# bluenote-1577/sylph

Measured on AMD Instinct MI355X. Metric: read Gbp/s sketched + genome-comparisons/s profiled, 1 Gbp vs GTDB-R220, higher is better.
Workload: dtype u64

## Files before the change

### sylph_amd/csrc/capi.hip

```cpp
#include <algorithm>
#include <memory>

#include <thread>

#include "common.h"

namespace sylph {

static thread_local char g_err[1024] = "";

void set_error(const char* fmt, ...) {
    va_list ap;
    va_start(ap, fmt);
    vsnprintf(g_err, sizeof(g_err), fmt, ap);
    va_end(ap);
}

ScopedKernelTimer::ScopedKernelTimer(sylph_ctx* c, const char* family) : ctx(c), fam(family) {
    if (!ctx->profile) return;
    if (!ctx->profile_only.empty()) {
        const size_t n = strlen(family);
        size_t at = 0;
        bool found = false;
        while ((at = ctx->profile_only.find(family, at)) != std::string::npos) {
// ... 372 lines not shown
    sylph::ctx_unref(ctx);
}

int sylph_ctx_set_option(sylph_ctx* ctx, const char* key, const char* value) {
    return guarded([&] {
        SY_REQUIRE(ctx && key && value, "null argument");
        std::lock_guard<std::mutex> lock(ctx->mu);
        if (!strcmp(key, "finish")) {
            if (!strcmp(value, "auto")) ctx->finish_mode = 0;
            else if (!strcmp(value, "generic")) ctx->finish_mode = 1;
            else if (!strcmp(value, "bucket")) ctx->finish_mode = 2;
            else SY_REQUIRE(false, "finish must be auto|generic|bucket");
        } else if (!strcmp(key, "seeds")) {
            if (!strcmp(value, "auto") || !strcmp(value, "ordered")) ctx->seeds_mode = 0;
            else if (!strcmp(value, "unordered")) ctx->seeds_mode = 1;
            else if (!strcmp(value, "slots")) ctx->seeds_mode = 2;
            else SY_REQUIRE(false, "seeds must be auto|slots|unordered");
        } else if (!strcmp(key, "bucket_target")) {
            const long v = strtol(value, nullptr, 10);
            SY_REQUIRE(v >= 16 && v <= 256, "bucket_target must be in [16, 256]");
            ctx->bucket_target = (uint32_t)v;
        } else if (!strcmp(key, "plain_records")) {
            ctx->plain_records = (uint32_t)strtol(value, nullptr, 10) ? 1u : 0u;
        } else if (!strcmp(key, "shard_reduce")) {
            if (!strcmp(value, "alltoall")) ctx->shard_reduce = 0;
            else if (!strcmp(value, "allgather")) ctx->shard_reduce = 1;
            else SY_REQUIRE(false, "shard_reduce must be alltoall|allgather");
        } else if (!strcmp(key, "stream_priority")) {
            SY_REQUIRE(ctx->own_stream, "stream_priority: the context runs on the caller's stream");
            int least = 0, greatest = 0;
            DeviceGuard dg(ctx->device);
            SY_HIP(hipDeviceGetStreamPriorityRange(&least, &greatest));
            int prio = 0;
            if (!strcmp(value, "high")) prio = greatest;
            else if (!strcmp(value, "low")) prio = least;
            else SY_REQUIRE(!strcmp(value, "normal"), "stream_priority must be high|normal|low");
            SY_HIP(hipStreamSynchronize(ctx->stream));
            hipStream_t s = nullptr;
            SY_HIP(hipStreamCreateWithPriority(&s, hipStreamNonBlocking, prio));
            (void)hipStreamDestroy(ctx->stream);
            ctx->stream = s;
        } else if (!strcmp(key, "fail_next_peer_copy")) {
            ctx->fail_next_peer_copy = (uint32_t)strtol(value, nullptr, 10);
        } else if (!strcmp(key, "fail_next_shard_probe")) {
            ctx->fail_next_shard_probe = (uint32_t)strtol(value, nullptr, 10);
        } else if (!strcmp(key, "push_chunk_bytes")) {
            const long long v = strtoll(value, nullptr, 10);
            SY_REQUIRE(v >= 64 && v <= (1ll << 31), "push_chunk_bytes must be in [64, 2^31]");
            ctx->push_chunk_bytes = (uint64_t)v;
        } else if (!strcmp(key, "reads_wg_per_cu")) {
            const long v = strtol(value, nullptr, 10);
            SY_REQUIRE(v >= 0 && v <= 64, "reads_wg_per_cu must be in [0, 64]");
            ctx->reads_wg_per_cu = (uint32_t)v;
        } else if (!strcmp(key, "profile_only")) {
            ctx->profile_only = (!value[0] || !strcmp(value, "all")) ? std::string() : "," + std::string(value) + ",";
        } else if (!strcmp(key, "reads_tail_pct")) {
            const long v = strtol(value, nullptr, 10);
            SY_REQUIRE(v >= 0 && v <= 50, "reads_tail_pct must be in [0, 50]");
            ctx->reads_tail_pct = (uint32_t)v;
        } else if (!strcmp(key, "reads_hash")) {
            const long v = strtol(value, nullptr, 10);
            SY_REQUIRE(v >= -1 && v <= 2, "reads_hash must be -1 (default), 0, 1 or 2");
            ctx->reads_hash = (int)v;
        } else if (!strcmp(key, "reads_slack")) {
            ctx->reads_slack = (uint32_t)strtoul(value, nullptr, 0);
        } else if (!strcmp(key, "index_lambda")) {
            const long v = strtol(value, nullptr, 10);
            SY_REQUIRE(v >= 1 && v <= 8, "index_lambda must be in [1, 8]");
            ctx->index_lambda = (uint32_t)v;
        } else if (!strcmp(key, "cu_mask")) {
            SY_REQUIRE(ctx->own_stream, "cu_mask: the context runs on a caller-supplied stream");
            int cus = 256;
            (void)hipDeviceGetAttribute(&cus, hipDeviceAttributeMultiprocessorCount, ctx->device);
            long lo = 0, hi = cus;
            if (strcmp(value, "all")) {
                char* end = nullptr;
                lo = strtol(value, &end, 10);
                SY_REQUIRE(end && *end == ':', "cu_mask must be lo:hi or all");
                hi = strtol(end + 1, nullptr, 10);
            }
            SY_REQUIRE(lo >= 0 && lo < hi && hi <= cus, "cu_mask range [%ld, %ld) outside the device's %d CUs", lo, hi, cus);
            DeviceGuard dg(ctx->device);
            SY_HIP(hipStreamSynchronize(ctx->stream));
            std::vector<uint32_t> mask((size_t)(cus + 31) / 32, 0u);
            for (long i = lo; i < hi; i++) mask[(size_t)i >> 5] |= 1u << (i & 31);
            hipStream_t ns = nullptr;
            SY_HIP(hipExtStreamCreateWithCUMask(&ns, (uint32_t)mask.size(), mask.data()));
            (void)hipStreamDestroy(ctx->stream);
            ctx->stream = ns;
        } else if (!strcmp(key, "index_pass_max")) {
            const long long v = strtoll(value, nullptr, 10);
            SY_REQUIRE(v >= 1 && v <= (1ll << 31), "index_pass_max must be in [1, 2^31]");
            ctx->index_pass_max = (uint64_t)v;
        } else {
            SY_REQUIRE(false, "unknown option %s", key);
        }
    });
}

int sylph_ctx_profile(sylph_ctx* ctx, int enable) {
    return guarded([&] {
        SY_REQUIRE(ctx, "null ctx");
        std::lock_guard<std::mutex> lock(ctx->mu);
        profile_collect(ctx);
        ctx->stats.clear();
        ctx->profile = enable != 0;
// ... 16 lines not shown
```

### sylph_amd/csrc/common.h

```cpp
#pragma once
#include <hip/hip_runtime.h>

#include <atomic>
#include <cstdarg>
#include <cstdint>
#include <cstdio>
#include <cstdlib>
#include <cstring>
#include <ctime>
#include <map>
#include <mutex>
#include <string>
#include <vector>

#include "../../include/sylph_hip.h"

struct sylph_ctx;

namespace sylph {

void set_error(const char* fmt, ...);

struct HipError { hipError_t e; const char* what; const char* file; int line; };

// ... 70 lines not shown
    void alloc(size_t want) {
        if (ctx) p = pool_acquire(ctx, want, &cap);
        else { SY_HIP(hipMalloc(&p, want)); cap = want; }
    }
    void reserve(size_t bytes) {
        if (bytes <= cap) return;
        release();
        alloc(bytes + bytes / 4 + 256);
    }
    void grow_keep(size_t bytes, size_t keep, hipStream_t s) {
        if (bytes <= cap) return;
        void* old = p;
        const size_t old_cap = cap;
        p = nullptr;
        cap = 0;
        alloc(bytes * 2 + 256);
        if (keep && old) SY_HIP(hipMemcpyAsync(p, old, keep, hipMemcpyDeviceToDevice, s));
        if (old) {
            if (ctx) pool_release(ctx, old, old_cap);
            else { SY_HIP(hipStreamSynchronize(s)); (void)hipFree(old); }
        }
    }
    template <class T> T* as() const { return reinterpret_cast<T*>(p); }
};

struct KernelStat { double ms = 0; uint64_t launches = 0; };

}

#ifndef SYLPH_READS_TAIL_PCT
#define SYLPH_READS_TAIL_PCT 10
#endif
struct sylph_ctx {
    int device = 0;
    hipStream_t stream = nullptr;
    bool own_stream = false;
    std::mutex mu;
    int finish_mode = 0;
    uint32_t bucket_target = 128;
    uint32_t plain_records = 1;
    uint32_t shard_reduce = 0;
    uint32_t fail_next_peer_copy = 0;
    uint32_t fail_next_shard_probe = 0;
    uint32_t index_lambda = 0;
    uint64_t index_pass_max = 1ull << 30;
    struct SeedTurn { hipEvent_t gate = nullptr, done = nullptr; bool recorded = false; } turn;
    void seed_gate() { if (turn.gate) { (void)hipStreamWaitEvent(stream, turn.gate, 0); turn.gate = nullptr; } }
    void seed_done() { if (turn.done && !turn.recorded && hipEventRecord(turn.done, stream) == hipSuccess) turn.recorded = true; }
    std::string profile_only;
    uint32_t reads_tail_pct = SYLPH_READS_TAIL_PCT;
    int reads_hash = -1;
    uint32_t reads_slack = 0;
    uint32_t reads_wg_per_cu = 0;
    uint64_t push_chunk_bytes = 64ull << 20;
    int seeds_mode = 0;
    std::atomic<int> refs{1};
    bool profile = false;
    std::map<std::string, sylph::KernelStat> stats;
    struct Pending { std::string fam; hipEvent_t a, b; };
    std::vector<Pending> pending;
    std::vector<hipEvent_t> event_pool;
    std::vector<std::pair<size_t, void*>> pool_free;
    size_t pool_bytes = 0;
    sylph::DevBuf tmp_sort;
    sylph::DevBuf scratch[8];
    sylph::DevBuf counters;
    void* pinned = nullptr;
    void read_back(void* dst, const void* dev_src, size_t bytes);
    static constexpr size_t STAGE_BYTES = 32u << 20;
    void* stage[2] = {nullptr, nullptr};
    hipEvent_t stage_ev[2] = {nullptr, nullptr};
    hipStream_t copy_stream = nullptr;
    hipEvent_t copy_ev[2] = {nullptr, nullptr};
    void d2h(void* dst, const void* dev_src, size_t bytes);
    void h2d(void* dev_dst, const void* src, size_t bytes);
};

namespace sylph {

struct ScopedKernelTimer {
    sylph_ctx* ctx;
    hipEvent_t a = nullptr, b = nullptr;
    const char* fam;
    ScopedKernelTimer(sylph_ctx* c, const char* family);
    ~ScopedKernelTimer();
};
void profile_collect(sylph_ctx* ctx);
void ctx_unref(sylph_ctx* ctx);

struct HostPhase {
    sylph_ctx* ctx;
    const char* name;
    double t0 = 0;
    static bool enabled() { static const bool e = getenv("SYLPH_HIP_TRACE") != nullptr; return e; }
    static double now() { timespec ts; clock_gettime(CLOCK_MONOTONIC, &ts); return ts.tv_sec * 1e3 + ts.tv_nsec * 1e-6; }
    HostPhase(sylph_ctx* c, const char* n) : ctx(c), name(n) { if (enabled()) { (void)hipStreamSynchronize(c->stream); t0 = now(); } }
    ~HostPhase() { if (enabled()) { (void)hipStreamSynchronize(ctx->stream); fprintf(stderr, "[sylph_hip] %-28s %8.3f ms\n", name, now() - t0); } }
};

struct DeviceGuard {
    int prev = -1;
    explicit DeviceGuard(int dev) {
        (void)hipGetDevice(&prev);
        if (prev != dev) SY_HIP(hipSetDevice(dev));
        else prev = -1;
    }
    ~DeviceGuard() { if (prev >= 0) (void)hipSetDevice(prev); }
};

void sort_pairs_u64_u32(sylph_ctx* ctx, const uint64_t* kin, uint64_t* kout, const uint32_t* vin, uint32_t* vout,
                        size_t n, int begin_bit, int end_bit);
void sort_pairs_u32_u64(sylph_ctx* ctx, const uint32_t* kin, uint32_t* kout, const uint64_t* vin, uint64_t* vout,
                        size_t n, int begin_bit, int end_bit);
void sort_pairs_u32_u32(sylph_ctx* ctx, const uint32_t* kin, uint32_t* kout, const uint32_t* vin, uint32_t* vout,
                        size_t n, int begin_bit, int end_bit);
constexpr uint32_t SPILL_MAX_TILES = 256;
struct SpillState { uint32_t n_tiles; uint32_t tiles[SPILL_MAX_TILES]; };
struct ReadsState { uint32_t long_record; SpillState spill; };

void sort_keys_u32(sylph_ctx* ctx, const uint32_t* kin, uint32_t* kout, size_t n, int begin_bit, int end_bit);
void sort_keys_u64(sylph_ctx* ctx, const uint64_t* kin, uint64_t* kout, size_t n, int begin_bit, int end_bit);
void exclusive_sum_u32(sylph_ctx* ctx, const uint32_t* in, uint32_t* out, size_t n);
void inclusive_max_u32(sylph_ctx* ctx, const uint32_t* in, uint32_t* out, size_t n);

inline int bit_length(uint64_t v) { int b = 0; while (v) { b++; v >>= 1; } return b; }

}
```

### sylph_amd/csrc/reads.hip

```cpp
#include <cstddef>

#include "common.h"
#include "device_common.h"
#include "sketch_session.h"

namespace sylph {

namespace {

constexpr int RTPB = 256;
constexpr int RT_MIN = 4096, RT_MAX = 65536;
constexpr int RH = 400;
constexpr int RPAD = 32;
constexpr int MASKW = 12;
constexpr int OFFS_256 = 600;
constexpr int RTPB_RAGGED = 512;

template <int K>
struct KC {
    static constexpr uint64_t MASK = (1ull << (2 * K)) - 1;
};

__device__ __forceinline__ uint64_t win64(const uint32_t* sF, uint32_t b) {
    const uint32_t j = b >> 4, ph = (b & 15u) * 2u;
// ... 28 lines not shown
    else { fhi = __builtin_amdgcn_alignbit(A0, A1, 32 - 2 * T); flo = __builtin_amdgcn_alignbit(A1, A2, 32 - 2 * T); }
    constexpr int OFF = 2 * T - D;
    if constexpr (OFF < 0) { rlo = __builtin_amdgcn_alignbit(B0, Bm, OFF + 32); rhi = __builtin_amdgcn_alignbit(B1, B0, OFF + 32); }
    else if constexpr (OFF == 0) { rlo = B0; rhi = B1; }
    else { rlo = __builtin_amdgcn_alignbit(B1, B0, OFF); rhi = __builtin_amdgcn_alignbit(B2, B1, OFF); }
    const uint64_t f = ((uint64_t)fhi << 32) | flo, rc = ((uint64_t)rhi << 32) | rlo;
    const uint64_t canon = (f < rc ? f : rc) >> D;
    if constexpr (HV == 2) {
        const uint32_t u = mm_hash64_gfx950_hi1(canon);
        asm("v_cmp_ge_u32 vcc, %2, %1\n\tv_addc_co_u32 %0, vcc, %0, %0, vcc" : "+v"(mask) : "v"(u), "s"((uint32_t)thr) : "vcc");
    } else {
        const uint64_t h = HV ? mm_hash64_gfx950(canon) : mm_hash64(canon);
        asm("v_cmp_lt_u64 vcc, %1, %2\n\tv_addc_co_u32 %0, vcc, %0, %0, vcc" : "+v"(mask) : "v"(h), "s"(thr) : "vcc");
    }
}
template <int K, int T0, int HV>
__device__ __forceinline__ void kmer_steps8(uint32_t A0, uint32_t A1, uint32_t A2, uint32_t Bm, uint32_t B0, uint32_t B1, uint32_t B2,
                                            uint64_t thr, uint32_t& mask) {
    kmer_step<K, T0 + 0, HV>(A0, A1, A2, Bm, B0, B1, B2, thr, mask);
    kmer_step<K, T0 + 1, HV>(A0, A1, A2, Bm, B0, B1, B2, thr, mask);
    kmer_step<K, T0 + 2, HV>(A0, A1, A2, Bm, B0, B1, B2, thr, mask);
    kmer_step<K, T0 + 3, HV>(A0, A1, A2, Bm, B0, B1, B2, thr, mask);
    kmer_step<K, T0 + 4, HV>(A0, A1, A2, Bm, B0, B1, B2, thr, mask);
    kmer_step<K, T0 + 5, HV>(A0, A1, A2, Bm, B0, B1, B2, thr, mask);
    kmer_step<K, T0 + 6, HV>(A0, A1, A2, Bm, B0, B1, B2, thr, mask);
    kmer_step<K, T0 + 7, HV>(A0, A1, A2, Bm, B0, B1, B2, thr, mask);
}

__global__ __launch_bounds__(256) void block_records_kernel(const uint64_t* __restrict__ off, uint64_t n_rec, uint32_t bias,
                                                            uint32_t rt, uint32_t n_entries, uint32_t* __restrict__ blk_rec,
                                                            uint32_t* __restrict__ count_sentinel, uint32_t* __restrict__ state_words) {
    const uint32_t b = blockIdx.x * blockDim.x + threadIdx.x;
    if (b == 0) { *count_sentinel = 0; state_words[0] = 0; state_words[1] = 0; }
    if (b >= n_entries) return;
    const uint64_t target = (uint64_t)b * rt;
    uint64_t lo = 0, hi = n_rec;
    while (lo < hi) {
        const uint64_t mid = (lo + hi) >> 1;
        if (off[mid] + bias < target) lo = mid + 1; else hi = mid;
    }
    blk_rec[b] = (uint32_t)lo;
}

#ifndef SYLPH_READS_HASH_DEFAULT
#define SYLPH_READS_HASH_DEFAULT 1
#endif
#ifndef SYLPH_READS_WAVES
#define SYLPH_READS_WAVES 5
#endif
template <int K, int HV, int ENC, int TPB>
__global__ __launch_bounds__(TPB) __attribute__((amdgpu_waves_per_eu(TPB == 256 ? SYLPH_READS_WAVES : 6, TPB == 256 ? SYLPH_READS_WAVES : 6))) void reads_kernel(const uint8_t* __restrict__ bases_al, uint32_t bias, uint64_t n_al,
                                                     const uint64_t* __restrict__ off, uint64_t n_rec,
                                                     const uint32_t* __restrict__ blk_rec, uint32_t n_blk, uint32_t it_begin, uint32_t it_end,
                                                     uint32_t rt, uint64_t thr,
                                                     uint32_t cand_slack, int avx2_compat, int paired, int want_markers, uint64_t rec_base,
                                                     uint32_t slot_cap, OccRec* __restrict__ slot_rec,
                                                     uint32_t* __restrict__ slot_key, int key_sh,
                                                     uint32_t* __restrict__ blk_count,
                                                     ReadsState* __restrict__ state, const uint32_t* __restrict__ blk_list,
                                                     uint32_t* __restrict__ spill_slot_of_blk) {
    constexpr int RTPB = TPB, OFFS = TPB == 256 ? OFFS_256 : 2 * TPB + 80;
    extern __shared__ uint32_t sF[];
    __shared__ uint64_t s_off[OFFS + 4];
    const uint32_t n_words = (rt + 2 * RH) / 16 + 3;
    __shared__ uint32_t s_mask[MASKW][RTPB];
    __shared__ uint32_t s_wave[RTPB / 64];
    static_assert((OFFS + 4) >= 2 * RTPB, "the marker arrays alias the staged offsets");
    uint64_t* const s_m0 = s_off;
    uint64_t* const s_m1 = s_off + RTPB;
    __shared__ uint32_t s_first[RTPB + 1], s_rel[RTPB];
    __shared__ uint16_t s_perm[RTPB], s_nh[RTPB];
    const uint32_t tid = threadIdx.x, lane = tid & 63, wave = tid >> 6;
    __shared__ uint32_t s_redo, s_redo_deal;
    const uint64_t thr_loop = HV == 2 ? (uint64_t)((uint32_t)(thr >> 32) + 1u + cand_slack) : thr;
    if (tid == 0) s_redo = 0;
    const uint32_t per_xcd = (n_blk + 7) / 8;
    for (uint32_t it0 = it_begin + blockIdx.x; it0 < it_end; it0 += gridDim.x) {
        const uint32_t it = blk_list ? it0 : (it0 & 7u) * per_xcd + (it0 >> 3);
        if (it >= n_blk) continue;
        const uint32_t blk = blk_list ? blk_list[it] : it;
        const int64_t a0 = (int64_t)blk * rt - RH;
        const bool interior = a0 >= 0 && (uint64_t)(a0 + (int64_t)n_words * 16) <= n_al;
        if (interior) {
            if constexpr (ENC == 0) {
                const uint4* __restrict__ src = reinterpret_cast<const uint4*>(bases_al + a0);
                for (uint32_t ci = tid; ci < n_words; ci += RTPB) sF[ci] = pack16_fwd(src[ci]);
            } else {
                const uint32_t* __restrict__ src = reinterpret_cast<const uint32_t*>(bases_al + (a0 >> 2));
                for (uint32_t ci = tid; ci < n_words; ci += RTPB) sF[ci] = __builtin_amdgcn_perm(0u, src[ci], 0x00010203u);
            }
        } else {
            for (uint32_t ci = tid; ci < n_words; ci += RTPB) {
                const int64_t a = a0 + (int64_t)ci * 16;
                if constexpr (ENC == 0) {
                    uint4 v = make_uint4(0, 0, 0, 0);
                    if (a >= 0 && (uint64_t)a < n_al) v = *reinterpret_cast<const uint4*>(bases_al + a);
                    sF[ci] = pack16_fwd(v);
                } else {
                    uint32_t w = 0;
                    if (a >= 0 && (uint64_t)a < n_al) w = *reinterpret_cast<const uint32_t*>(bases_al + (a >> 2));
                    sF[ci] = __builtin_amdgcn_perm(0u, w, 0x00010203u);
                }
            }
        }
        const uint64_t R0 = blk_rec[blk], R1 = blk_rec[blk + 1];
        const uint64_t w_lo = paired ? (R0 & ~1ull) : R0;
        const uint64_t w_hi = min(R1 + 2, n_rec);
        const bool in_lds = (w_hi - w_lo + 1) <= (uint64_t)(OFFS + 4) && (R1 - R0) <= (uint64_t)RTPB;
        if (in_lds)
            for (uint64_t t = tid; t <= w_hi - w_lo; t += RTPB) s_off[t] = off[w_lo + t];
        __syncthreads();
        uint32_t base_prev = 0;
        const uint64_t out0 = (uint64_t)it * slot_cap;
        for (uint64_t pass = R0; pass < R1; pass += RTPB) {
            const uint64_t r = pass + tid;
            const bool active = r < R1;
            uint64_t start = 0, L = 0, s1 = 0, s2 = 0, e2 = 0;
            if (active) {
                if (in_lds) {
                    start = s_off[r - w_lo];
                    L = s_off[r + 1 - w_lo] - start;
                    if (paired) { const uint64_t r1 = (r & ~1ull) - w_lo; s1 = s_off[r1]; s2 = s_off[r1 + 1]; e2 = s_off[r1 + 2]; }
                } else {
                    start = off[r];
                    L = off[r + 1] - start;
                    if (paired) { const uint64_t r1 = r & ~1ull; s1 = off[r1]; s2 = off[r1 + 1]; e2 = off[r1 + 2]; }
                }
            }
            const bool too_long = active && (L > (uint64_t)RH || (paired && (s2 - s1 > (uint64_t)RH || e2 - s2 > (uint64_t)RH)));
            if (too_long) state->long_record = 1u;
            const uint32_t nh = (active && !too_long) ? (uint32_t)n_hashed_kmers(L, K, avx2_compat, 0) : 0u;
            const uint32_t rel = active ? (uint32_t)((int64_t)(start + bias) - a0) : 0u;
            uint32_t* const s_hist = s_first;
            if (tid < 64) s_hist[tid] = 0;
            s_rel[tid] = rel;
            s_nh[tid] = (uint16_t)nh;
#ifndef SYLPH_READS_ALWAYS_DEAL
            if (tid == 0) s_redo_deal = 0;
            __syncthreads();
            if (__ballot(nh != (uint32_t)s_nh[0]) && lane == 0) s_redo_deal = 1;
            __syncthreads();
            const bool dealt = s_redo_deal != 0;
            const uint32_t bin = 63u - ((nh + 7) >> 3);
            uint32_t hg_max = (nh + 7) >> 3, arrival = 0, hc = 0;
            if (dealt) {
                arrival = atomicAdd(&s_hist[bin], 1u);
                __syncthreads();
                hc = s_hist[lane];
                const uint64_t bins_used = __ballot(hc != 0u);
                hg_max = bins_used ? 63u - (uint32_t)(__ffsll((unsigned long long)bins_used) - 1) : 0u;
            }
#else
            __syncthreads();
            const uint32_t bin = 63u - ((nh + 7) >> 3);
            const uint32_t arrival = atomicAdd(&s_hist[bin], 1u);
            __syncthreads();
            const uint32_t hc = s_hist[lane];
            const bool dealt = s_hist[bin] != (uint32_t)RTPB;
            const uint64_t bins_used = __ballot(hc != 0u);
            const uint32_t hg_max = bins_used ? 63u - (uint32_t)(__ffsll((unsigned long long)bins_used) - 1) : 0u;
#endif
            const uint32_t rows_used = min((uint32_t)MASKW, (hg_max * 8u + 31u) >> 5);
            if (dealt) {
                const uint32_t incl = wave_inclusive_sum(hc);
                s_perm[(uint32_t)__shfl((int)(incl - hc), (int)bin) + arrival] = (uint16_t)tid;
                __syncthreads();
            }
            const uint32_t slot = dealt ? s_perm[tid] : tid;
            const uint32_t rel_h = dealt ? s_rel[slot] : rel, nh_h = dealt ? s_nh[slot] : nh;
            uint32_t nh_max = nh_h;
#pragma unroll
            for (int d = 32; d > 0; d >>= 1) nh_max = max(nh_max, (uint32_t)__shfl_xor((int)nh_max, d));
            if (nh_max) {
                const uint32_t w0 = rel_h >> 4, sh = 32u - (rel_h & 15u) * 2u;
                uint32_t raw = sF[w0], nxt = sF[w0 + 1];
                auto next_word = [&](uint32_t j) {
                    const uint32_t a = (uint32_t)((((uint64_t)raw << 32) | nxt) >> sh);
                    raw = nxt;
                    nxt = sF[w0 + j + 2];
                    return a;
                };
                uint32_t A0 = next_word(0), A1 = next_word(1), A2 = next_word(2);
                uint32_t Bm = 0, B0 = rcword(A0), B1 = rcword(A1), B2 = rcword(A2);
                const uint32_t n_half = (nh_max + 7) >> 3;
                uint16_t* const mask_half = reinterpret_cast<uint16_t*>(&s_mask[0][slot]);
                const uint32_t n_grp = n_half >> 1;
                for (uint32_t g = 0; g < n_grp; g++) {
                    uint32_t mask = 0;
                    kmer_steps8<K, 0, HV>(A0, A1, A2, Bm, B0, B1, B2, thr_loop, mask);
                    kmer_steps8<K, 8, HV>(A0, A1, A2, Bm, B0, B1, B2, thr_loop, mask);
                    A0 = A1; A1 = A2; A2 = next_word(g + 3);
                    Bm = B0; B0 = B1; B1 = B2; B2 = rcword(A2);
                    mask_half[((g >> 1) * RTPB * 2) + ((g & 1u) ^ 1u)] = (uint16_t)mask;
                }
                if (n_half & 1u) {
                    uint32_t mask = 0;
                    kmer_steps8<K, 0, HV>(A0, A1, A2, Bm, B0, B1, B2, thr_loop, mask);
                    mask_half[((n_grp >> 1) * RTPB * 2) + ((n_grp & 1u) ^ 1u)] = (uint16_t)(mask << 8);
                }
            }
            if (dealt) __syncthreads();
            uint32_t total = 0;
            for (;;) {
            uint32_t cnt = 0;
            const uint32_t nw = (nh + 31) >> 5;
            for (uint32_t w = 0; w + 1 < nw; w++) cnt += __popc(s_mask[w][tid]);
            if (nw) {
                const uint32_t left = nh - (nw - 1) * 32;
                const uint32_t m = s_mask[nw - 1][tid] & (uint32_t)(0xFFFFFFFF00000000ull >> left);
                s_mask[nw - 1][tid] = m;
                cnt += __popc(m);
            }
            const uint32_t x = wave_inclusive_sum(cnt);
            __syncthreads();
            if (lane == 63) s_wave[wave] = x;
            __syncthreads();
            uint32_t before = 0;
            total = 0;
#pragma unroll
            for (int w = 0; w < RTPB / 64; w++) {
                const uint32_t t = s_wave[w];
                if ((uint32_t)w < wave) before += t;
                total += t;
            }
            {
                uint64_t m0 = 0, m1 = 0;
                uint32_t has = 0;
                if (cnt && want_markers) {
                    uint32_t ba = 0, bb = 0;
                    if (!paired) {
                        if (L >= 66 && L <= 400) { has = 1; ba = rel; bb = rel + (uint32_t)(L / 2); }
                    } else if (s2 - s1 >= 33 && e2 - s2 >= 33) {
                        has = 1;
                        ba = (uint32_t)((int64_t)(s1 + bias) - a0);
                        bb = (uint32_t)((int64_t)(s2 + bias) - a0);
                    }
                    if (has) {
                        const uint64_t wa64 = win64(sF, ba), wb64 = win64(sF, bb);
                        uint32_t ea, oa, eb, ob;
                        evenodd16(wa64, ea, oa);
                        evenodd16(wb64, eb, ob);
                        m0 = (uint64_t)ea | ((uint64_t)eb << 32);
                        m1 = (uint64_t)oa | ((uint64_t)ob << 32);
                    }
                }
                s_m0[tid] = m0;
                s_m1[tid] = m1;
                s_first[tid] = (before + x - cnt) | (has << 31);
                if (tid == 0) s_first[RTPB] = total;
            }
            uint32_t* const s_owner = &s_mask[0][0] + rows_used * RTPB;
            const bool listed = total <= ((uint32_t)MASKW - rows_used) * (uint32_t)RTPB;
            if (listed && cnt) {
                uint32_t p = before + x - cnt;
                for (uint32_t w = 0; w < nw; w++) {
                    uint32_t m = s_mask[w][tid];
                    while (m) {
                        const uint32_t bpos = (uint32_t)__clz((int)m);
                        s_owner[p++] = tid | ((w * 32 + bpos) << 10);
                        m &= ~(0x80000000u >> bpos);
                    }
                }
            }
            __syncthreads();
            for (uint32_t hix = tid; hix < total; hix += RTPB) {
                uint32_t lo, i = 0, f;
                if (listed) {
                    const uint32_t ow = s_owner[hix];
                    lo = ow & 0x3FFu;
                    i = ow >> 10;
                    f = s_first[lo];
                } else {
                    lo = 0;
                    uint32_t hi = RTPB;
                    while (hi - lo > 1) {
                        const uint32_t mid = (lo + hi) >> 1;
                        if ((s_first[mid] & 0x7FFFFFFFu) <= hix) lo = mid; else hi = mid;
                    }
                    f = s_first[lo];
                    uint32_t j = hix - (f & 0x7FFFFFFFu);
                    for (uint32_t w = 0; w < MASKW; w++) {
                        uint32_t m = s_mask[w][lo];
                        const uint32_t c = (uint32_t)__popc(m);
                        if (j >= c) { j -= c; continue; }
                        for (; j; j--) m &= ~(0x80000000u >> __clz((int)m));
                        i = w * 32 + (uint32_t)__clz((int)m);
                        break;
                    }
                }
                const uint32_t o = base_prev + hix;
                if (o < slot_cap) {
                    const uint64_t ft = win64(sF, s_rel[lo] + i);
                    const uint64_t fk = ft >> (64 - 2 * K), rk = revcomp_top<K>(ft);
#ifndef SYLPH_READS_COOP_PLAIN_HASH
                    const uint64_t h = mm_hash64_gfx950(fk < rk ? fk : rk);
#else
                    const uint64_t h = mm_hash64(fk < rk ? fk : rk);
#endif
                    if constexpr (HV == 2) {
                        if (h >= thr) {
                            atomicAnd(&s_mask[i >> 5][lo], ~(0x80000000u >> (i & 31u)));
                            s_redo = 1u;
                            continue;
                        }
                    }
                    uint64_t rid = rec_base + pass + lo;
                    if (f >> 31) {
                        rid |= RID_MARKER_BIT;
                        if (paired) rid |= min(emission_rank(i, s_nh[lo], avx2_compat), RID_RANK_MAX) << RID_RANK_SHIFT;
                    }
                    slot_rec[out0 + o] = OccRec{h, rid, s_m0[lo], s_m1[lo]};
                    if (slot_key) slot_key[out0 + o] = (uint32_t)(h >> key_sh);
                }
            }
            __syncthreads();
            if constexpr (HV != 2) break;
            else {
                if (!s_redo) break;
                __syncthreads();
                if (tid == 0) s_redo = 0;
            }
            }
            base_prev += total;
        }
        if (tid == 0) {
            if (blk_list) {
                spill_slot_of_blk[blk] = it;
            } else {
                blk_count[blk] = base_prev;
                if (base_prev > slot_cap) {
                    const uint32_t s = atomicAdd(&state->spill.n_tiles, 1u);
                    if (s < SPILL_MAX_TILES) state->spill.tiles[s] = blk;
                }
            }
        }
        __syncthreads();
    }
}

__global__ __launch_bounds__(64) void compact_occ_kernel(const OccRec* __restrict__ slot_rec, const uint32_t* __restrict__ blk_count,
                                                         const uint32_t* __restrict__ blk_off, uint32_t n_blk, uint32_t slot_cap,
                                                         uint32_t spill_cap, const OccRec* __restrict__ spill_rec,
                                                         const uint32_t* __restrict__ spill_slot_of_blk,
                                                         uint64_t* __restrict__ out_hash, OccRec* __restrict__ out_rec) {
    for (uint32_t b = blockIdx.x; b < n_blk; b += gridDim.x) {
        const uint32_t n = blk_count[b], d = blk_off[b];
        const OccRec* sr = slot_rec + (uint64_t)b * slot_cap;
        if (n > slot_cap) sr = spill_rec + (uint64_t)spill_slot_of_blk[b] * spill_cap;
        for (uint32_t i = threadIdx.x; i < n; i += blockDim.x) {
            const OccRec r = sr[i];
            out_hash[d + i] = r.hash;
            out_rec[d + i] = r;
        }
    }
}

uint32_t grid_for(uint64_t n, uint32_t tpb = 256) { return (uint32_t)((n + tpb - 1) / tpb); }

__global__ __launch_bounds__(1024) void block_total_kernel(const uint32_t* __restrict__ blk_count, uint32_t n_blk, uint32_t* __restrict__ total) {
    __shared__ uint32_t s[16];
    uint32_t v = 0;
    for (uint32_t i = threadIdx.x; i < n_blk; i += 1024) v += blk_count[i];
#pragma unroll
    for (int d = 32; d > 0; d >>= 1) v += (uint32_t)__shfl_xor((int)v, d);
    if ((threadIdx.x & 63) == 0) s[threadIdx.x >> 6] = v;
    __syncthreads();
    if (threadIdx.x == 0) {
        uint32_t t = 0;
        for (int w = 0; w < 16; w++) t += s[w];
        *total = t;
    }
}

struct SlotMeta {
    uint32_t *blk_rec, *blk_count, *spill_slot, *blk_off;
    ReadsState* state;
    SlotMeta(sylph_sketch* sk, uint32_t n_blk) {
        blk_rec = sk->slot_meta.as<uint32_t>();
        blk_count = blk_rec + (n_blk + 1);
        spill_slot = blk_count + (n_blk + 1);
        blk_off = spill_slot + (n_blk + 1);
        state = reinterpret_cast<ReadsState*>(blk_off + (n_blk + 1));
    }
};

void compact_region(sylph_sketch* sk, uint32_t n_blk, uint32_t slot_cap, uint32_t n, uint32_t spill_cap, const OccRec* spill_rec) {
    sylph_ctx* ctx = sk->ctx;
    SlotMeta m(sk, n_blk);
    exclusive_sum_u32(ctx, m.blk_count, m.blk_off, (size_t)n_blk + 1);
    const uint64_t need = sk->n_occ + n;
    sk->hash.grow_keep(need * 8, sk->n_occ * 8, ctx->stream);
    sk->recs.grow_keep(need * sizeof(OccRec), sk->n_occ * sizeof(OccRec), ctx->stream);
    {
        ScopedKernelTimer t(ctx, "compact");
        hipLaunchKernelGGL(compact_occ_kernel, dim3(std::min<uint32_t>(n_blk, 1u << 16)), dim3(64), 0, ctx->stream,
                           sk->slot_rec.as<OccRec>(), m.blk_count, m.blk_off, n_blk, slot_cap, spill_cap, spill_rec, m.spill_slot,
                           sk->hash.as<uint64_t>() + sk->n_occ, sk->recs.as<OccRec>() + sk->n_occ);
        SY_HIP(hipGetLastError());
    }
    sk->n_occ = need;
}

}

void resolve_deferred_slots(sylph_sketch* sk) {
    if (!sk->pend.live || !sk->pend.deferred) return;
    sylph_ctx* ctx = sk->ctx;
    SlotMeta m(sk, sk->pend.n_blk);
    hipLaunchKernelGGL(block_total_kernel, dim3(1), dim3(1024), 0, ctx->stream, m.blk_count, sk->pend.n_blk, m.blk_off + sk->pend.n_blk);
    uint32_t res[3] = {0, 0, 0};
    ctx->read_back(res, m.blk_off + sk->pend.n_blk, 12);
    if (res[1] || res[2]) { redo_deferred_batch(sk); return; }
    sk->pend.deferred = false;
    sk->pend.n = res[0];
    if (res[0] == 0) sk->pend = PendingSlots{};
}

void flush_pending_slots(sylph_sketch* sk) {
    resolve_deferred_slots(sk);
    if (!sk->pend.live) return;
    compact_region(sk, sk->pend.n_blk, sk->pend.slot_cap, sk->pend.n, 0, nullptr);
    sk->pend = PendingSlots{};
}

bool push_short_reads(sylph_sketch* sk, const uint8_t* d_bases, uint32_t phase, const uint64_t* d_off, uint64_t n_records, uint64_t n_bases,
                      int enc) {
    sylph_ctx* ctx = sk->ctx;
    const uint32_t bias = enc == SYLPH_ENC_2BIT ? (uint32_t)((uintptr_t)d_bases & 15) * 4u + phase : (uint32_t)((uintptr_t)d_bases & 15);
    const uint8_t* bases_al = d_bases - ((uintptr_t)d_bases & 15);
    const uint64_t n_al = n_bases + bias;
    static const int env_ragged_tpb = [] { const char* e = getenv("SYLPH_HIP_READS_RAGGED_TPB"); return e ? atoi(e) : RTPB; }();
    const bool ragged = (n_bases % n_records) != 0;
    const int tpb = (ragged && env_ragged_tpb == RTPB_RAGGED && (uint64_t)RTPB_RAGGED * 93 / 100 * n_bases / n_records <= (uint64_t)RT_MAX) ? RTPB_RAGGED : RTPB;
    const uint64_t target = ragged ? (uint64_t)tpb * 93 / 100 : (uint64_t)tpb;
    uint32_t rt = (uint32_t)std::min<uint64_t>(RT_MAX, std::max<uint64_t>(RT_MIN, target * n_bases / n_records));
    rt = (rt + 15u) & ~15u;
    const uint32_t n_blk = (uint32_t)(n_al / rt) + 1;
    const uint64_t expect = (uint64_t)rt / sk->c;
    const uint32_t spill_cap = rt + RH;
    const uint32_t slot_cap = (uint32_t)std::min<uint64_t>(spill_cap, expect + expect * 3 / 4 + 48);
    const size_t lds_bytes = ((size_t)(rt + 2 * RH) / 16 + 3 + RPAD) * 4;
    const uint64_t thr = UINT64_MAX / (uint64_t)sk->c;
    sk->slot_rec.reserve((size_t)n_blk * slot_cap * sizeof(OccRec));
    sk->slot_key.reserve((size_t)n_blk * slot_cap * 4);
    sk->slot_meta.reserve(((size_t)n_blk + 1) * 4 * 4 + sizeof(ReadsState) + 16);
    SlotMeta m(sk, n_blk);
    static_assert(offsetof(ReadsState, long_record) == 0 && offsetof(ReadsState, spill) == 4 && offsetof(SpillState, n_tiles) == 0,
                  "long_record and spill.n_tiles are the first two words");
    int cus = 256;
    (void)hipDeviceGetAttribute(&cus, hipDeviceAttributeMultiprocessorCount, ctx->device);
    static const int hv_env = getenv("SYLPH_HIP_HASH_VARIANT") ? atoi(getenv("SYLPH_HIP_HASH_VARIANT")) : SYLPH_READS_HASH_DEFAULT;
    const int hv_want = ctx->reads_hash >= 0 ? ctx->reads_hash : hv_env;
    const uint32_t slack = ctx->reads_slack;
    const int hv = (hv_want == 2 && ((thr >> 32) + 1ull + slack) > 0xFFFFFFFFull) ? 1 : hv_want;
    const int key_sh = key_shift(sk->c);
    auto launch = [&](uint32_t n_it, uint32_t it_b, uint32_t it_e, uint32_t cap, OccRec* sr, uint32_t* skey, const uint32_t* list) {
        if (it_e <= it_b) return;
        const uint32_t grid = ctx->reads_wg_per_cu ? (uint32_t)std::min<uint64_t>(it_e - it_b, (uint64_t)cus * ctx->reads_wg_per_cu) : it_e - it_b;
#define SY_LAUNCH_READS_T(KK, HH, EE, TT)                                                                                             \
    hipLaunchKernelGGL((reads_kernel<KK, HH, EE, TT>), dim3(grid), dim3(TT), lds_bytes, ctx->stream, bases_al, bias, n_al, d_off, n_records, \
                       m.blk_rec, n_it, it_b, it_e, rt, thr, slack, sk->avx2_compat, sk->paired, sk->no_dedup ? 0 : 1, sk->rec_base, cap, sr, skey, key_sh,   \
                       m.blk_count, m.state, list, m.spill_slot)
#define SY_LAUNCH_READS(KK, HH, EE) do { if (tpb == RTPB_RAGGED) SY_LAUNCH_READS_T(KK, HH, EE, RTPB_RAGGED); else SY_LAUNCH_READS_T(KK, HH, EE, RTPB); } while (0)
        if (enc == SYLPH_ENC_2BIT) {
            if (sk->k == 31) { if (hv == 2) SY_LAUNCH_READS(31, 2, 1); else SY_LAUNCH_READS(31, 1, 1); }
            else { if (hv == 2) SY_LAUNCH_READS(21, 2, 1); else SY_LAUNCH_READS(21, 1, 1); }
        } else if (sk->k == 31) { if (hv == 2) SY_LAUNCH_READS(31, 2, 0); else if (hv) SY_LAUNCH_READS(31, 1, 0); else SY_LAUNCH_READS(31, 0, 0); }
        else { if (hv == 2) SY_LAUNCH_READS(21, 2, 0); else if (hv) SY_LAUNCH_READS(21, 1, 0); else SY_LAUNCH_READS(21, 0, 0); }
#undef SY_LAUNCH_READS_T
#undef SY_LAUNCH_READS
        SY_HIP(hipGetLastError());
    };
    {
        HostPhase ph(ctx, "push: reads kernel");
        {
            ScopedKernelTimer t(ctx, "annotate");
            hipLaunchKernelGGL(block_records_kernel, dim3(grid_for(n_blk + 1)), dim3(256), 0, ctx->stream, d_off, n_records, bias, rt,
                               n_blk + 1, m.blk_rec, m.blk_count + n_blk, reinterpret_cast<uint32_t*>(m.state));
        }
        ctx->seed_gate();
        {
            const uint32_t n_round = ((n_blk + 7) / 8) * 8;
            uint32_t cut = n_round;
            if (ctx->turn.done && !ctx->turn.recorded && ctx->reads_tail_pct && n_round >= 64)
                cut = (uint32_t)((uint64_t)n_round * (100 - ctx->reads_tail_pct) / 100) & ~7u;
            {
                ScopedKernelTimer t(ctx, "seeds");
                launch(n_blk, 0, cut, slot_cap, sk->slot_rec.as<OccRec>(), sk->slot_key.as<uint32_t>(), nullptr);
            }
            ctx->seed_done();
            if (cut < n_round) {
                ScopedKernelTimer t(ctx, "seeds");
                launch(n_blk, cut, n_round, slot_cap, sk->slot_rec.as<OccRec>(), sk->slot_key.as<uint32_t>(), nullptr);
            }
        }
        const uint64_t n_expect = (n_bases > n_records * (uint64_t)(sk->k - 1) ? n_bases - n_records * (uint64_t)(sk->k - 1) : 0) / sk->c;
        if (sk->borrow_until_finish && sk->n_occ == 0 && sk->rec_base == 0 && ctx->finish_mode == 0 && sk->c >= 2 && n_expect >= 4096 &&
            (uint64_t)n_blk * slot_cap < (1ull << 31)) {
            sk->pend = PendingSlots{};
            sk->pend.live = true;
            sk->pend.deferred = true;
            sk->pend.n_blk = n_blk;
            sk->pend.slot_cap = slot_cap;
            sk->pend.n = n_blk * slot_cap;
            sk->pend.n_expect = (uint32_t)std::min<uint64_t>(n_expect, sk->pend.n);
            sk->pend.bases = d_bases; sk->pend.phase = phase; sk->pend.off = d_off;
            sk->pend.n_records = n_records; sk->pend.n_bases = n_bases; sk->pend.enc = enc;
            if (ctx->profile) ctx->stats["deferred"].launches++;
            return true;
        }
        hipLaunchKernelGGL(block_total_kernel, dim3(1), dim3(1024), 0, ctx->stream, m.blk_count, n_blk, m.blk_off + n_blk);
    }
    uint32_t res[3] = {0, 0, 0};
    SY_HIP(hipMemcpyAsync(ctx->pinned, m.blk_off + n_blk, 12, hipMemcpyDeviceToHost, ctx->stream));
    SY_HIP(hipStreamSynchronize(ctx->stream));
    memcpy(res, ctx->pinned, 12);
    if (!ctx->pending.empty()) profile_collect(ctx);
    if (res[1] || res[2] > SPILL_MAX_TILES) return false;
    const uint32_t n = res[0];
    if (n == 0) return true;
    if (res[2] == 0 && sk->n_occ == 0 && ctx->finish_mode != 1 && sk->c >= 2) {
        sk->pend.live = true;
        sk->pend.n_blk = n_blk;
        sk->pend.slot_cap = slot_cap;
        sk->pend.n = n;
        return true;
    }
    const OccRec* sp_r = nullptr;
    if (res[2]) {
        DevBuf& b_x = ctx->scratch[7];
        b_x.reserve((size_t)res[2] * spill_cap * sizeof(OccRec));
        OccRec* xr = b_x.as<OccRec>();
        ScopedKernelTimer ts(ctx, "seeds_spill");
        ScopedKernelTimer t(ctx, "seeds");
        launch(res[2], 0, res[2], spill_cap, xr, nullptr, m.state->spill.tiles);
        sp_r = xr;
    }
    compact_region(sk, n_blk, slot_cap, n, spill_cap, sp_r);
    return true;
}

}
```

### sylph_amd/csrc/replay_lds.hip

```cpp
#include "common.h"
#include "device_common.h"
#include "sketch_session.h"
#include "partition.h"

namespace sylph {
namespace {

#ifndef SYLPH_REPLAY_TPB
#define SYLPH_REPLAY_TPB 128
#endif
constexpr int CAP_SMALL = 256, RTPB_SMALL = SYLPH_REPLAY_TPB;
constexpr int CAP_MID = 512, RTPB_MID = 256;
constexpr int CAP_LARGE = 1024, RTPB_LARGE = 256;
constexpr int IDX_BITS = 10;
constexpr uint32_t SEG_LIMIT = 96;


struct ReplayArgs {
    const OccRec* recs;
    const uint64_t* hash;
    const uint32_t* perm;
    const uint32_t* boff;
    const uint32_t* p_nv;
    int paired, dedup;
// ... 877 lines not shown
    uint32_t* chunk_rows = mid_list + (B + 2) + ((B & 1u) ? 1 : 0);
    unsigned long long* chunk_removed = reinterpret_cast<unsigned long long*>(chunk_rows + 264);
    FinishTail* d_tail = b_small.as<FinishTail>();
    const uint32_t* d_nv = boff + B;
    const uint32_t n_zero = (B + 2) * 2;
    const int dbg = getenv("SYLPH_REPLAY_STAGE") ? atoi(getenv("SYLPH_REPLAY_STAGE")) : 0;
    const uint32_t cutoff = sk->paired ? 0u : 4u;
    sk->out_k.reserve((size_t)n_cap * 8);
    sk->out_c.reserve((size_t)n_cap * 4);
    ReplayArgs ra{};
    if (plain) ra.hash = sorted_hash;
    else { ra.recs = recs; ra.perm = b_perm.as<uint32_t>(); }
    ra.boff = boff; ra.p_nv = d_nv;
    ra.paired = sk->paired; ra.dedup = sk->dedup_mode(); ra.cutoff = cutoff; ra.bm = bm;
    ra.tmp_k = b_tmpk.as<uint64_t>(); ra.tmp_c = b_tmpc.as<uint32_t>(); ra.n_distinct = n_distinct; ra.removed_b = removed_b;
    ra.overflow = &d_tail->overflow;
    ra.mid_list = mid_list; ra.large_list = large_list; ra.ovf_list = ovf_list; ra.dbg_stage = dbg;
    {
        HostPhase ph(ctx, "finish(bucket): partition + LDS replay + compact");
        {
            ScopedKernelTimer t(ctx, "sort");
            launch_partition(ctx, in, bm, geom, n_tiles, n_all, hist, pairs, boff, b_perm.as<uint32_t>(), sorted_hash, n_distinct, n_zero,
                             b_small.as<uint32_t>(), large_list, ovf_list, mid_list);
        }
        {
            ScopedKernelTimer t(ctx, "replay");
            if (plain) hipLaunchKernelGGL((bucket_count_kernel<CAP_SMALL, RTPB_SMALL>), dim3(B), dim3(RTPB_SMALL), 0, ctx->stream, ra);
            else hipLaunchKernelGGL((bucket_replay_kernel<CAP_SMALL, RTPB_SMALL>), dim3(B), dim3(RTPB_SMALL), 0, ctx->stream, ra);
        }
    }
    auto close_table = [&](int skip_if_listed) {
        const uint32_t ipt = (B + (1u << 18) - 1) >> 18;
        ScopedKernelTimer t(ctx, "replay");
        hipLaunchKernelGGL(table_scan_kernel, dim3((B + SCAN_CHUNK * ipt - 1) / (SCAN_CHUNK * ipt)), dim3(SCAN_CHUNK), 0, ctx->stream, n_distinct,
                           removed_b, B, ipt, d_off, chunk_rows, chunk_removed);
        hipLaunchKernelGGL(table_compact_kernel, dim3(std::min<uint32_t>((B + 3) / 4, 1u << 15)), dim3(256), 0, ctx->stream,
                           b_tmpk.as<uint64_t>(), b_tmpc.as<uint32_t>(), boff, d_off, chunk_rows, chunk_removed, n_distinct, B, ipt,
                           sk->out_k.as<uint64_t>(), sk->out_c.as<uint32_t>(), ovf_list, mid_list, large_list, skip_if_listed,
                           d_tail, deferred ? sk->slot_meta.as<uint32_t>() + (size_t)(sk->pend.n_blk + 1) * 4 : (const uint32_t*)nullptr,
                           sk->a10_state == 1 ? sk->a10_tail.as<uint32_t>() : (const uint32_t*)nullptr, d_nv);
        SY_HIP(hipGetLastError());
    };
    FinishTail host{};
    auto read_tail = [&] {
        SY_HIP(hipMemcpyAsync(ctx->pinned, d_tail, sizeof host, hipMemcpyDeviceToHost, ctx->stream));
        SY_HIP(hipStreamSynchronize(ctx->stream));
        memcpy(&host, ctx->pinned, sizeof host);
        if (!ctx->pending.empty()) profile_collect(ctx);
    };
    close_table(1);
    read_tail();
    if (deferred) {
        if (host.verdict[0] || host.verdict[1]) {
            redo_deferred_batch(sk);
            a10_mark(sk);
            return finish_bucketed(sk);
        }
        sk->pend.deferred = false;
        sk->pend.n = host.n_found;
    }
    if (!a10_verdict(sk, host.a10_words)) return finish_bucketed(sk);
    if (host.overflow) return false;
    if (plain && host.n_ovf) {
        materialise_plain_records(sk);
        return finish_bucketed(sk);
    }
    if (host.n_mid || host.n_large) {
        HostPhase ph(ctx, "finish(bucket): medium / large configurations");
        {
            ScopedKernelTimer t(ctx, "replay");
            if (plain) {
                if (host.n_large)
                    hipLaunchKernelGGL((bucket_count_list_kernel<CAP_LARGE, RTPB_LARGE>), dim3(std::min<uint32_t>(host.n_large, 1536u)),
                                       dim3(RTPB_LARGE), 0, ctx->stream, ra, large_list);
            } else {
                if (host.n_mid)
                    hipLaunchKernelGGL((bucket_replay_list_kernel<CAP_MID, RTPB_MID>), dim3(std::min<uint32_t>(host.n_mid, 1280u)),
                                       dim3(RTPB_MID), 0, ctx->stream, ra, mid_list);
                if (host.n_large)
                    hipLaunchKernelGGL((bucket_replay_list_kernel<CAP_LARGE, RTPB_LARGE>), dim3(std::min<uint32_t>(host.n_large, 512u)),
                                       dim3(RTPB_LARGE), 0, ctx->stream, ra, large_list);
            }
        }
        close_table(0);
        read_tail();
        if (host.overflow) return false;
    }
    unsigned long long removed_extra = 0;
    if (host.n_ovf) {
        if (ctx->finish_mode == 2 || host.n_ovf > 4096) return false;
        HostPhase ph(ctx, "finish(bucket): overflowing buckets through the device-wide path");
        const uint32_t m = host.n_ovf;
        DevBuf b_so(ctx), b_si(ctx), b_sh(ctx), b_sr(ctx), sub_k(ctx), sub_c(ctx);
        b_so.reserve(((size_t)m + 1) * 4);
        hipLaunchKernelGGL(ovf_offsets_kernel, dim3(1), dim3(1024), 0, ctx->stream, ovf_list, boff, b_so.as<uint32_t>());
        uint32_t n_sub = 0;
        ctx->read_back(&n_sub, b_so.as<uint32_t>() + m, 4);
        b_si.reserve((size_t)n_sub * 8);
        b_sh.reserve((size_t)n_sub * 8);
        b_sr.reserve((size_t)n_sub * sizeof(OccRec));
        uint32_t* sub_idx = b_si.as<uint32_t>();
        uint32_t* sub_sorted = sub_idx + n_sub;
        hipLaunchKernelGGL(ovf_indices_kernel, dim3(m), dim3(256), 0, ctx->stream, ovf_list, b_so.as<uint32_t>(), boff,
                           b_perm.as<uint32_t>(), sub_idx);
        sort_keys_u32(ctx, sub_idx, sub_sorted, n_sub, 0, 32);
        {
// ... 22 lines not shown
```

### sylph_amd/csrc/sketch_session.h

```cpp
#pragma once
#include <algorithm>

#include "common.h"

namespace sylph {
constexpr uint64_t RID_MARKER_BIT = 1ull << 63;
constexpr uint64_t RID_A10_BIT = 1ull << 62;
constexpr int RID_RANK_SHIFT = 42;
constexpr uint64_t RID_RANK_MAX = (1ull << 20) - 1;
constexpr uint64_t RID_MASK = (1ull << RID_RANK_SHIFT) - 1;
constexpr uint64_t INVALID_HASH = ~0ull;
struct alignas(32) OccRec { uint64_t hash, rid, m0, m1; };
}

namespace sylph {
void flush_pending_slots(sylph_sketch* sk);
inline int key_shift(uint32_t c) { return std::max(0, bit_length(UINT64_MAX / (uint64_t)std::max<uint32_t>(c, 1)) - 32); }
constexpr int DEDUP_EXACT = 0, DEDUP_NONE = 1, DEDUP_FILTER = 2;
void generic_replay(sylph_ctx* ctx, const uint64_t* d_hash, const OccRec* d_recs, uint32_t n_all, bool paired, int dedup,
                    DevBuf& out_k, DevBuf& out_c, uint64_t& n_out, uint64_t& removed_out);
void a10_mark(sylph_sketch* sk);
void a10_settle(sylph_sketch* sk);
bool a10_verdict(sylph_sketch* sk, const uint32_t words[2]);
void materialise_plain_records(sylph_sketch* sk);
}

namespace sylph {
struct PendingSlots {
    bool live = false;
    uint32_t n_blk = 0, slot_cap = 0, n = 0;
    bool deferred = false;
    uint32_t n_expect = 0;
    const uint8_t* bases = nullptr;
    uint32_t phase = 0;
    const uint64_t* off = nullptr;
    uint64_t n_records = 0, n_bases = 0;
    int enc = 0;
};
void resolve_deferred_slots(sylph_sketch* sk);
void redo_deferred_batch(sylph_sketch* sk);
}

struct sylph_sketch {
    sylph_ctx* ctx;
    uint32_t c, k;
    int paired, no_dedup, avx2_compat;
    bool finished = false;
    bool borrow_until_finish = false;
    double dedup_fpr = 0.;
    uint64_t dedup_capacity = 10000000;
    int a10_state = 0;
    int a10_force = 0;
    bool filter_dedup() const { return paired && !no_dedup && dedup_fpr > 0.; }
    int dedup_mode() const { return no_dedup ? sylph::DEDUP_NONE : (filter_dedup() ? sylph::DEDUP_FILTER : sylph::DEDUP_EXACT); }
    uint64_t rec_base = 0;
    uint64_t n_occ = 0;
    uint64_t n_plain = 0;
    sylph::DevBuf hash;
    sylph::DevBuf recs;
    sylph::DevBuf slot_bases[2], slot_off[2];
    sylph::DevBuf slot_rec, slot_key, slot_meta;
    sylph::PendingSlots pend;
    sylph::DevBuf batch_ascii;
    sylph::DevBuf fq_bases, fq_off;
    sylph::DevBuf out_k, out_c;
    uint64_t n_out = 0, dup_removed = 0;
    sylph::DevBuf counters;
    sylph::DevBuf a10_tail;
    explicit sylph_sketch(sylph_ctx* cx)
        : ctx(cx), hash(cx), recs(cx), slot_bases{sylph::DevBuf(cx), sylph::DevBuf(cx)}, slot_off{sylph::DevBuf(cx), sylph::DevBuf(cx)},
          slot_rec(cx), slot_key(cx), slot_meta(cx), batch_ascii(cx), fq_bases(cx), fq_off(cx), out_k(cx), out_c(cx), counters(cx), a10_tail(cx) {}
};
```

Before: 1103.

## Size read-kernel mask LDS dynamically from mean read length

Replaces the fixed static shared mask array of MASKW rows in the reads kernel with a dynamically sized region. The row count comes from the batch's mean read length, the expected hit count, and the longest k-mer count seen so far. Records needing more rows than fit set a verdict word, and the host then relearns the size and relaunches the batch. The aim is to cut LDS use per workgroup for short reads so more workgroups stay resident, at the cost of occasional redo launches and an extra atomic per record.

```diff
diff --git a/sylph_amd/csrc/capi.hip b/sylph_amd/csrc/capi.hip
--- a/sylph_amd/csrc/capi.hip
+++ b/sylph_amd/csrc/capi.hip
@@ -448,6 +448,10 @@
             const long v = strtol(value, nullptr, 10);
             SY_REQUIRE(v >= 0 && v <= 64, "reads_wg_per_cu must be in [0, 64]");
             ctx->reads_wg_per_cu = (uint32_t)v;
+        } else if (!strcmp(key, "reads_mask_rows")) {
+            const long v = strtol(value, nullptr, 10);
+            SY_REQUIRE(v >= 0 && v <= 12, "reads_mask_rows must be in [0, 12]");
+            ctx->reads_mask_rows = (uint32_t)v;
         } else if (!strcmp(key, "profile_only")) {
             ctx->profile_only = (!value[0] || !strcmp(value, "all")) ? std::string() : "," + std::string(value) + ",";
         } else if (!strcmp(key, "reads_tail_pct")) {
diff --git a/sylph_amd/csrc/common.h b/sylph_amd/csrc/common.h
--- a/sylph_amd/csrc/common.h
+++ b/sylph_amd/csrc/common.h
@@ -146,6 +146,8 @@
     int reads_hash = -1;
     uint32_t reads_slack = 0;
     uint32_t reads_wg_per_cu = 0;
+    uint32_t reads_mask_rows = 0;
+    uint32_t reads_nh_seen = 0;
     uint64_t push_chunk_bytes = 64ull << 20;
     int seeds_mode = 0;
     std::atomic<int> refs{1};
@@ -211,6 +213,7 @@
 constexpr uint32_t SPILL_MAX_TILES = 256;
 struct SpillState { uint32_t n_tiles; uint32_t tiles[SPILL_MAX_TILES]; };
 struct ReadsState { uint32_t long_record; SpillState spill; };
+constexpr uint32_t READS_LONG_BIT = 0x80000000u;
 
 void sort_keys_u32(sylph_ctx* ctx, const uint32_t* kin, uint32_t* kout, size_t n, int begin_bit, int end_bit);
 void sort_keys_u64(sylph_ctx* ctx, const uint64_t* kin, uint64_t* kout, size_t n, int begin_bit, int end_bit);
diff --git a/sylph_amd/csrc/reads.hip b/sylph_amd/csrc/reads.hip
--- a/sylph_amd/csrc/reads.hip
+++ b/sylph_amd/csrc/reads.hip
@@ -104,7 +104,7 @@
 __global__ __launch_bounds__(TPB) __attribute__((amdgpu_waves_per_eu(TPB == 256 ? SYLPH_READS_WAVES : 6, TPB == 256 ? SYLPH_READS_WAVES : 6))) void reads_kernel(const uint8_t* __restrict__ bases_al, uint32_t bias, uint64_t n_al,
                                                      const uint64_t* __restrict__ off, uint64_t n_rec,
                                                      const uint32_t* __restrict__ blk_rec, uint32_t n_blk, uint32_t it_begin, uint32_t it_end,
-                                                     uint32_t rt, uint64_t thr,
+                                                     uint32_t rt, uint32_t mask_rows, uint32_t fit_rows, uint64_t thr,
                                                      uint32_t cand_slack, int avx2_compat, int paired, int want_markers, uint64_t rec_base,
                                                      uint32_t slot_cap, OccRec* __restrict__ slot_rec,
                                                      uint32_t* __restrict__ slot_key, int key_sh,
@@ -112,10 +112,11 @@
                                                      ReadsState* __restrict__ state, const uint32_t* __restrict__ blk_list,
                                                      uint32_t* __restrict__ spill_slot_of_blk) {
     constexpr int RTPB = TPB, OFFS = TPB == 256 ? OFFS_256 : 2 * TPB + 80;
-    extern __shared__ uint32_t sF[];
+    extern __shared__ uint32_t s_dyn[];
     __shared__ uint64_t s_off[OFFS + 4];
     const uint32_t n_words = (rt + 2 * RH) / 16 + 3;
-    __shared__ uint32_t s_mask[MASKW][RTPB];
+    uint32_t* const s_mask = s_dyn;
+    uint32_t* const sF = s_dyn + mask_rows * RTPB;
     __shared__ uint32_t s_wave[RTPB / 64];
     static_assert((OFFS + 4) >= 2 * RTPB, "the marker arrays alias the staged offsets");
     uint64_t* const s_m0 = s_off;
@@ -180,8 +181,11 @@
                 }
             }
             const bool too_long = active && (L > (uint64_t)RH || (paired && (s2 - s1 > (uint64_t)RH || e2 - s2 > (uint64_t)RH)));
-            if (too_long) state->long_record = 1u;
-            const uint32_t nh = (active && !too_long) ? (uint32_t)n_hashed_kmers(L, K, avx2_compat, 0) : 0u;
+            if (too_long) atomicOr(&state->long_record, READS_LONG_BIT);
+            const uint32_t nh_rec = (active && !too_long) ? (uint32_t)n_hashed_kmers(L, K, avx2_compat, 0) : 0u;
+            const bool too_wide = nh_rec > fit_rows * 32u;
+            if (too_wide) atomicMax(&state->long_record, nh_rec);
+            const uint32_t nh = too_wide ? 0u : nh_rec;
             const uint32_t rel = active ? (uint32_t)((int64_t)(start + bias) - a0) : 0u;
             uint32_t* const s_hist = s_first;
             if (tid < 64) s_hist[tid] = 0;
@@ -212,7 +216,7 @@
             const uint64_t bins_used = __ballot(hc != 0u);
             const uint32_t hg_max = bins_used ? 63u - (uint32_t)(__ffsll((unsigned long long)bins_used) - 1) : 0u;
 #endif
-            const uint32_t rows_used = min((uint32_t)MASKW, (hg_max * 8u + 31u) >> 5);
+            const uint32_t rows_used = min(mask_rows, (hg_max * 8u + 31u) >> 5);
             if (dealt) {
                 const uint32_t incl = wave_inclusive_sum(hc);
                 s_perm[(uint32_t)__shfl((int)(incl - hc), (int)bin) + arrival] = (uint16_t)tid;
@@ -235,7 +239,7 @@
                 uint32_t A0 = next_word(0), A1 = next_word(1), A2 = next_word(2);
                 uint32_t Bm = 0, B0 = rcword(A0), B1 = rcword(A1), B2 = rcword(A2);
                 const uint32_t n_half = (nh_max + 7) >> 3;
-                uint16_t* const mask_half = reinterpret_cast<uint16_t*>(&s_mask[0][slot]);
+                uint16_t* const mask_half = reinterpret_cast<uint16_t*>(s_mask + slot);
                 const uint32_t n_grp = n_half >> 1;
                 for (uint32_t g = 0; g < n_grp; g++) {
                     uint32_t mask = 0;
@@ -256,11 +260,11 @@
             for (;;) {
             uint32_t cnt = 0;
             const uint32_t nw = (nh + 31) >> 5;
-            for (uint32_t w = 0; w + 1 < nw; w++) cnt += __popc(s_mask[w][tid]);
+            for (uint32_t w = 0; w + 1 < nw; w++) cnt += __popc(s_mask[w * RTPB + tid]);
             if (nw) {
                 const uint32_t left = nh - (nw - 1) * 32;
-                const uint32_t m = s_mask[nw - 1][tid] & (uint32_t)(0xFFFFFFFF00000000ull >> left);
-                s_mask[nw - 1][tid] = m;
+                const uint32_t m = s_mask[(nw - 1) * RTPB + tid] & (uint32_t)(0xFFFFFFFF00000000ull >> left);
+                s_mask[(nw - 1) * RTPB + tid] = m;
                 cnt += __popc(m);
             }
             const uint32_t x = wave_inclusive_sum(cnt);
@@ -301,12 +305,12 @@
                 s_first[tid] = (before + x - cnt) | (has << 31);
                 if (tid == 0) s_first[RTPB] = total;
             }
-            uint32_t* const s_owner = &s_mask[0][0] + rows_used * RTPB;
-            const bool listed = total <= ((uint32_t)MASKW - rows_used) * (uint32_t)RTPB;
+            uint32_t* const s_owner = s_mask + rows_used * RTPB;
+            const bool listed = total <= (mask_rows - rows_used) * (uint32_t)RTPB;
             if (listed && cnt) {
                 uint32_t p = before + x - cnt;
                 for (uint32_t w = 0; w < nw; w++) {
-                    uint32_t m = s_mask[w][tid];
+                    uint32_t m = s_mask[w * RTPB + tid];
                     while (m) {
                         const uint32_t bpos = (uint32_t)__clz((int)m);
                         s_owner[p++] = tid | ((w * 32 + bpos) << 10);
@@ -331,8 +335,8 @@
                     }
                     f = s_first[lo];
                     uint32_t j = hix - (f & 0x7FFFFFFFu);
-                    for (uint32_t w = 0; w < MASKW; w++) {
-                        uint32_t m = s_mask[w][lo];
+                    for (uint32_t w = 0; w < mask_rows; w++) {
+                        uint32_t m = s_mask[w * RTPB + lo];
                         const uint32_t c = (uint32_t)__popc(m);
                         if (j >= c) { j -= c; continue; }
                         for (; j; j--) m &= ~(0x80000000u >> __clz((int)m));
@@ -351,7 +355,7 @@
 #endif
                     if constexpr (HV == 2) {
                         if (h >= thr) {
-                            atomicAnd(&s_mask[i >> 5][lo], ~(0x80000000u >> (i & 31u)));
+                            atomicAnd(&s_mask[(i >> 5) * RTPB + lo], ~(0x80000000u >> (i & 31u)));
                             s_redo = 1u;
                             continue;
                         }
@@ -455,6 +459,13 @@
 
 }
 
+bool learn_reads_verdict(sylph_ctx* ctx, uint32_t word) {
+    if (word == 0 || (word & READS_LONG_BIT)) return false;
+    ctx->reads_nh_seen = std::max(ctx->reads_nh_seen, word);
+    if (ctx->profile) ctx->stats["reads_regrow"].launches++;
+    return true;
+}
+
 void resolve_deferred_slots(sylph_sketch* sk) {
     if (!sk->pend.live || !sk->pend.deferred) return;
     sylph_ctx* ctx = sk->ctx;
@@ -462,7 +473,7 @@
     hipLaunchKernelGGL(block_total_kernel, dim3(1), dim3(1024), 0, ctx->stream, m.blk_count, sk->pend.n_blk, m.blk_off + sk->pend.n_blk);
     uint32_t res[3] = {0, 0, 0};
     ctx->read_back(res, m.blk_off + sk->pend.n_blk, 12);
-    if (res[1] || res[2]) { redo_deferred_batch(sk); return; }
+    if (res[1] || res[2]) { learn_reads_verdict(ctx, res[1]); redo_deferred_batch(sk); return; }
     sk->pend.deferred = false;
     sk->pend.n = res[0];
     if (res[0] == 0) sk->pend = PendingSlots{};
@@ -491,7 +502,22 @@
     const uint64_t expect = (uint64_t)rt / sk->c;
     const uint32_t spill_cap = rt + RH;
     const uint32_t slot_cap = (uint32_t)std::min<uint64_t>(spill_cap, expect + expect * 3 / 4 + 48);
-    const size_t lds_bytes = ((size_t)(rt + 2 * RH) / 16 + 3 + RPAD) * 4;
+    uint32_t fit_rows, mask_rows;
+    {
+        const uint64_t mean_len = (n_bases + n_records - 1) / n_records;
+        const uint32_t nh_cap = (uint32_t)std::min<uint64_t>(MASKW * 32, std::max<uint64_t>({1, n_hashed_kmers(mean_len, (uint32_t)sk->k, sk->avx2_compat, 0), ctx->reads_nh_seen}));
+        fit_rows = (nh_cap + 31) / 32;
+        if (ctx->reads_mask_rows) {
+            fit_rows = mask_rows = std::min<uint32_t>(MASKW, std::max(ctx->reads_mask_rows, (ctx->reads_nh_seen + 31) / 32));
+        } else {
+            const uint64_t hits = (uint64_t)tpb * nh_cap / sk->c;
+            const uint32_t avail = MASKW - fit_rows;
+            uint32_t list_rows = (uint32_t)((hits + hits / 2 + 32 + tpb - 1) / tpb);
+            if (list_rows > avail) list_rows = (hits + tpb - 1) / tpb <= avail ? avail : 0;
+            mask_rows = fit_rows + list_rows;
+        }
+    }
+    const size_t lds_bytes = ((size_t)(rt + 2 * RH) / 16 + 3 + RPAD + (size_t)mask_rows * tpb) * 4;
     const uint64_t thr = UINT64_MAX / (uint64_t)sk->c;
     sk->slot_rec.reserve((size_t)n_blk * slot_cap * sizeof(OccRec));
     sk->slot_key.reserve((size_t)n_blk * slot_cap * 4);
@@ -511,7 +537,7 @@
         const uint32_t grid = ctx->reads_wg_per_cu ? (uint32_t)std::min<uint64_t>(it_e - it_b, (uint64_t)cus * ctx->reads_wg_per_cu) : it_e - it_b;
 #define SY_LAUNCH_READS_T(KK, HH, EE, TT)                                                                                             \
     hipLaunchKernelGGL((reads_kernel<KK, HH, EE, TT>), dim3(grid), dim3(TT), lds_bytes, ctx->stream, bases_al, bias, n_al, d_off, n_records, \
-                       m.blk_rec, n_it, it_b, it_e, rt, thr, slack, sk->avx2_compat, sk->paired, sk->no_dedup ? 0 : 1, sk->rec_base, cap, sr, skey, key_sh,   \
+                       m.blk_rec, n_it, it_b, it_e, rt, mask_rows, fit_rows, thr, slack, sk->avx2_compat, sk->paired, sk->no_dedup ? 0 : 1, sk->rec_base, cap, sr, skey, key_sh,   \
                        m.blk_count, m.state, list, m.spill_slot)
 #define SY_LAUNCH_READS(KK, HH, EE) do { if (tpb == RTPB_RAGGED) SY_LAUNCH_READS_T(KK, HH, EE, RTPB_RAGGED); else SY_LAUNCH_READS_T(KK, HH, EE, RTPB); } while (0)
         if (enc == SYLPH_ENC_2BIT) {
@@ -568,6 +594,7 @@
     SY_HIP(hipStreamSynchronize(ctx->stream));
     memcpy(res, ctx->pinned, 12);
     if (!ctx->pending.empty()) profile_collect(ctx);
+    if (learn_reads_verdict(ctx, res[1])) return push_short_reads(sk, d_bases, phase, d_off, n_records, n_bases, enc);
     if (res[1] || res[2] > SPILL_MAX_TILES) return false;
     const uint32_t n = res[0];
     if (n == 0) return true;
diff --git a/sylph_amd/csrc/replay_lds.hip b/sylph_amd/csrc/replay_lds.hip
--- a/sylph_amd/csrc/replay_lds.hip
+++ b/sylph_amd/csrc/replay_lds.hip
@@ -953,6 +953,7 @@
     read_tail();
     if (deferred) {
         if (host.verdict[0] || host.verdict[1]) {
+            learn_reads_verdict(ctx, host.verdict[0]);
             redo_deferred_batch(sk);
             a10_mark(sk);
             return finish_bucketed(sk);
diff --git a/sylph_amd/csrc/sketch_session.h b/sylph_amd/csrc/sketch_session.h
--- a/sylph_amd/csrc/sketch_session.h
+++ b/sylph_amd/csrc/sketch_session.h
@@ -37,6 +37,7 @@
     uint64_t n_records = 0, n_bases = 0;
     int enc = 0;
 };
+bool learn_reads_verdict(sylph_ctx* ctx, uint32_t word);
 void resolve_deferred_slots(sylph_sketch* sk);
 void redo_deferred_batch(sylph_sketch* sk);
 }
```

Result: no change. 1107, median of 6 (+0.3%).
